# 959AI994/Multi-Gate-VAE

Measured on AMD Instinct MI355X. Metric: circuit-graphs/sec (train step), AIG-64k batch=64 per GPU, higher is better.
Workload: dtype f32 storage; dense products as bf16x3 split-precision MFMA, fp32 accumulate; 1 GPU; cfg2: DG_AE --type aig, 64 x 65536-node synthetic levelised DAGs per GPU (N=4194304, E=6558720, 120 levels), H=64, 4+4 rounds, layernorm, weights [1,4,4], negatives sampled; step includes the 7-scalar metrics copy (pinned, read one step behind); global_batch=64, parallelism=dp1

## Files before the change

### include/mgvae_hip.h

```cpp
#ifndef MGVAE_HIP_H
#define MGVAE_HIP_H
#include <stdint.h>
#ifdef __cplusplus
extern "C" {
#endif

#ifndef MGV_OK
#define MGV_OK 0
#define MGV_EINVAL (-1)
#define MGV_EUNSUPPORTED (-2)
#endif

int mgv_abi_version(void);

int mgv_struct_stage_fwd(int H, int64_t N, const float* h_in, const int32_t* nbr_ptr, const int32_t* nbr_idx,
                         const uint8_t* xcls, const float* xtab, int C, const float* Wc, const float* bc,
                         const float* Whh, const float* bhh, const float* ln_w, const float* ln_b, float ln_eps,
                         float* h_out, void* stream);
int mgv_struct_stage_bwd(int H, int64_t N, const float* h_in, const int32_t* nbr_ptr, const int32_t* nbr_idx,
                         const uint8_t* xcls, const float* xtab, int C, const float* Wc, const float* WcT,
                         const float* bc, const float* Whh, const float* WhhT, const float* bhh,
                         const float* ln_w, const float* ln_b, float ln_eps, const float* gy_direct,
                         const float* gy_agg, float* g_direct_out, float* g_agg_out, float* dWc, float* dbc,
                         float* dWhh, float* dbhh, float* dxtab, float* dln_w, float* dln_b, void* stream);
int mgv_struct_stage_rows_fwd(int H, int64_t N, const float* h_in, const int32_t* nbr_ptr, const int32_t* nbr_idx,
                              const float* xrow, const float* Wc, const float* bc, const float* Whh, const float* bhh,
                              const float* ln_w, const float* ln_b, float ln_eps, float* h_out, void* stream);
int mgv_struct_stage_rows_bwd(int H, int64_t N, const float* h_in, const int32_t* nbr_ptr, const int32_t* nbr_idx,
                              const float* xrow, const float* Wc, const float* WcT, const float* bc, const float* Whh,
                              const float* WhhT, const float* bhh, const float* ln_w, const float* ln_b, float ln_eps,
                              const float* gy_direct, const float* gy_agg, float* g_direct_out, float* g_agg_out,
                              float* dWc, float* dbc, float* dWhh, float* dbhh, float* d_xrow, float* dln_w, float* dln_b,
                              void* stream);

int mgv_struct_stage_fwd_x3(int H, int64_t N, const float* h_in, const int32_t* nbr_ptr, const int32_t* nbr_idx,
                            const uint8_t* xcls, const float* xtab, int C, const void* wpack_bf16, const float* bc,
                            const float* bhh, const float* ln_w, const float* ln_b, float ln_eps, float* h_out,
                            int heavy_n, const int32_t* heavy_nodes, float* heavy_ws, const int32_t* table_own_idx,
                            int nbr_tagged, float* ln_stats_out, void* stream);
int mgv_struct_stage_bwd_x3(int H, int64_t N, const float* h_in, const int32_t* nbr_ptr, const int32_t* nbr_idx,
                            const uint8_t* xcls, const float* xtab, int C, const void* wpack_bf16, const float* bc,
                            const float* bhh, const float* ln_w, const float* ln_b, float ln_eps,
                            const float* gy_direct, const float* gy_agg, float* g_direct_out, float* g_agg_out,
                            float* dWc, float* dbc, float* dWhh, float* dbhh, float* dxtab, float* dln_w,
                            float* dln_b, int heavy_n, const int32_t* heavy_nodes, float* heavy_ws, const int32_t* table_own_idx,
                            int nbr_tagged, void* stream);

int mgv_struct_stage_bwd2_ws_floats(int H, int64_t N);
int mgv_struct_stage_bwd2_x3(int H, int64_t N, const float* h_in, const int32_t* nbr_ptr, const int32_t* nbr_idx,
                             const uint8_t* xcls, const float* xtab, int C, const void* wpack_bf16, const float* bc,
                             const float* bhh, const float* ln_w, const float* ln_b, float ln_eps,
                             const float* gy_direct, const float* gy_agg, float* g_direct_out, float* g_agg_out,
                             float* dWc, float* dbc, float* dWhh, float* dbhh, float* dxtab, float* dln_w,
                             float* dln_b, float* workspace, int64_t workspace_floats, int heavy_n,
                             const int32_t* heavy_nodes, float* heavy_ws, const int32_t* table_own_idx,
                             int nbr_tagged, const float* ln_stats, void* stream);

int mgv_linear_fwd(int64_t N, const float* X1, int K1, int ld1, const float* X2, int K2, int ld2,
                   const float* W, const float* b, int M, float* Y, int ldy, void* stream);
int mgv_linear_wgrad(int64_t N, const float* X1, int K1, int ld1, const float* X2, int K2, int ld2,
                     const float* dY, int lddy, int M, float* dW, float* db, void* stream);
int mgv_linear_x3_supported(int M, int K);
int mgv_wpack_bf16x3(const float* W, int R, int K, int ldw, int transpose, void* hi, void* lo, void* stream);
int mgv_linear_fwd_x3(int64_t N, const float* X1, int K1, int ld1, const float* X2, int K2, int ld2,
                      const void* wpack_bf16, const float* b, int M, float* Y, int ldy, void* stream);
int mgv_grouped_linear_supported(int M, int K);
int mgv_grouped_linear_fwd_x3(int64_t ntiles, const int32_t* tile_list, const int32_t* order, const int32_t* tile_start,
                              const int32_t* tile_count, const int32_t* tile_slot, const float* X, int K, int ldx,
                              const void* wpack_bf16, const float* b, int M, const float* R, int ldr, float* Y, int ldy, void* stream);
int mgv_grouped_linear_wgrad_x3_ws_floats(int M, int K, int64_t ntiles);
int mgv_grouped_linear_wgrad_x3(int64_t ntiles, const int32_t* tile_list, const int32_t* order, const int32_t* tile_start,
                                const int32_t* tile_count, const float* X, int K, int ldx, const float* dY, int lddy, int M,
                                float* dW, float* db, float* workspace, int64_t workspace_floats, void* stream);
int mgv_linear_fwd_x3_res(int64_t N, const float* X1, int K1, int ld1, const float* X2, int K2, int ld2,
                          const void* wpack_bf16, const float* b, int M, const float* R, int ldr, float* Y, int ldy,
                          void* stream);
int mgv_linear_wgrad_x3_ws_floats(int M, int K, int64_t N);
int mgv_linear_wgrad_x3(int64_t N, const float* X1, int K1, int ld1, const float* X2, int K2, int ld2,
                        const float* dY, int lddy, int M, float* dW, float* db, float* workspace, int64_t workspace_floats,
                        void* stream);
int mgv_linear_bwd_x3_supported(int M, int K);
int mgv_linear_bwd_x3(int64_t N, const float* X1, int K1, int ld1, const float* X2, int K2, int ld2, const float* dY, int lddy,
                      int M, const void* wtpack_bf16, float* dW, float* db, float* dX1, int ldx1, float* dX2, int ldx2,
                      const float* R, int ldr, float* workspace, int64_t workspace_floats, void* stream);
int mgv_gather_sum(int H, int64_t N, const float* h, const int32_t* nbr_ptr, const int32_t* nbr_idx,
                   float* agg, float* deg, void* stream);

int mgv_class_expand(int H, int64_t N, const float* table, const int32_t* class_id, float* out, void* stream);
int mgv_seg_sum(int H, int64_t n_seg, const int32_t* seg_ptr, const int32_t* items, const float* direct, const float* agg,
                const int32_t* nbr_ptr, const int32_t* nbr_idx, const int32_t* out_row, float* out, void* stream);
int mgv_seg_sum_entries(int H, int64_t n_seg, const int32_t* seg_ptr, const int32_t* entries, const float* direct, const float* agg,
                        const int32_t* out_row, float* out, void* stream);

int mgv_class_pull_sum_ws_floats(int H, int64_t N, int C);
int mgv_class_pull_sum(int H, int64_t N, const float* gy_direct, const float* gy_agg, const int32_t* nbr_ptr,
                       const int32_t* nbr_idx, const int32_t* class_id, int C, float* out, float* workspace,
                       int64_t workspace_floats, void* stream);

int mgv_func_sweep_fwd(int H, int64_t N, int T, int num_levels, const int32_t* level_tile_ptr_host,
                       const int32_t* order, const int32_t* tile_start, const int32_t* tile_count,
                       const int32_t* tile_slot, const int32_t* in_ptr, const int32_t* in_src, const float* hs,
                       float* hf, const float* attn_u, const float* Wvc, const float* bvc, const float* bih,
                       const float* bhh, const float* gh, const float* h_prev, void* stream);
int mgv_func_sweep_bwd(int H, int64_t N, int T, int num_levels, const int32_t* level_tile_ptr_host,
                       const int32_t* order, const int32_t* tile_start, const int32_t* tile_count,
                       const int32_t* tile_slot, const int32_t* in_ptr, const int32_t* in_src,
                       const int32_t* out_ptr, const int32_t* out_dst, const int32_t* out_slot,
                       const uint8_t* gslot, const float* hs, const float* hf, const float* attn_u,
                       const float* Wvc, const float* WvcT, const float* bvc, const float* bih, const float* bhh,
                       const float* ghf, float* ghs, float* dzb, float* alpha, float* dsc, float* d_attn_u,
                       float* dWvc, float* dbvc, float* dbih, float* dbhh, const float* gh, const float* h_prev,
                       float* d_gh, float* g_hprev, void* stream);

int mgv_sweep_zero_inactive(int H, int64_t N, const uint8_t* gslot, float* hf, void* stream);
int mgv_func_sweep_fwd_x3(int H, int64_t N, int T, int num_levels, const int32_t* level_tile_ptr_host,
                          const int32_t* order, const int32_t* order_span, int order_span_ints, const int32_t* tile_start,
                          const int32_t* tile_count, const int32_t* tile_slot, const int32_t* in_ptr,
                          const int32_t* in_src, const float* hs, float* hf, const float* attn_u,
                          const void* wpack_bf16, const float* bvc, const float* bih, const float* bhh,
                          const float* gh, const float* h_prev, void* stream);
int mgv_func_sweep_bwd_x3(int H, int64_t N, int T, int num_levels, const int32_t* level_tile_ptr_host,
                          const int32_t* order, const int32_t* order_span, int order_span_ints, int64_t n_active,
                          const int32_t* tile_start, const int32_t* tile_count, const int32_t* tile_slot,
                          const int32_t* slot_tiles, const int32_t* slot_tile_ptr_host, const int32_t* in_ptr,
                          const int32_t* in_src, const int32_t* out_ptr, const int32_t* out_dst,
                          const int32_t* out_slot, const uint8_t* gslot, const float* hs, const float* hf,
                          const float* attn_u, const void* wpack_bf16, const float* bvc, const float* bih,
                          const float* bhh, const float* ghf, float* ghs, float* dzb, float* alpha, float* dsc,
                          float* d_attn_u, float* dWvc, float* dbvc, float* dbih, float* dbhh, float* scratch,
                          int64_t scratch_elems,
                          int skip_inactive_longer_than ,
                          int heavy_active_n, const int32_t* heavy_nodes, const int32_t* heavy_node_seg_ptr, const int32_t* heavy_seg_e0,
                          const int32_t* heavy_seg_e1, const int32_t* heavy_lvl_k_ptr_host, const int32_t* heavy_lvl_seg_ptr_host,
                          float* heavy_ws, int skip_active_longer_than,
                          const float* gh, const float* h_prev, float* d_gh, float* g_hprev, void* stream);

int mgv_attn_pool_fwd(int W, int64_t N, const int32_t* in_ptr, const int32_t* in_src, const float* x, const float* u,
                      float* zbar, float* mstat, float* inv, void* stream);
int mgv_attn_pool_bwd(int W, int64_t N, const int32_t* in_ptr, const int32_t* in_src, const float* x, const float* u,
                      const float* zbar, const float* mstat, const float* inv, const float* dzbar, float* dx, float* du,
                      void* stream);

int mgv_sweep_pull_heavy(int H, int K, const int32_t* nodes, const int32_t* node_seg_ptr, int S, const int32_t* seg_e0,
                         const int32_t* seg_e1, const int32_t* out_dst, const int32_t* out_slot, const uint8_t* gslot,
                         const float* alpha, const float* dsc, const float* dzb, const float* attn_u, float* partial_ws,
                         float* ghs, void* stream);

int mgv_edge_dot_fwd(int H, int64_t E, const float* s, const float* t, int ld, const int64_t* src,
                     const int64_t* dst, int sigmoid, float* out, void* stream);
int mgv_edge_dot_bwd(int H, int64_t E, const float* s, const float* t, int ld, const int64_t* src,
                     const int64_t* dst, int sigmoid, const float* gout, float* ds, float* dt, void* stream);
int mgv_pair_scores_fwd(int H, int64_t M, int64_t N, const float* s, int lds, const float* t, int ldt, int sigmoid, float* out,
                        int64_t ldo, void* stream);
int mgv_pair_scores_bwd(int H, int64_t M, int64_t N, const float* s, int lds, const float* t, int ldt, int sigmoid, const float* out,
                        int64_t ldo, const float* gout, int64_t ldg, float* ds, int ldds, float* dt, int lddt, void* stream);
int mgv_pair_scores_at(int H, int64_t E, const float* s, int lds, const float* t, int ldt, const int64_t* src, const int64_t* dst,
                       int sigmoid, float* out, void* stream);
int mgv_pair_topk(int H, int64_t N, const float* s, int lds, const float* t, int ldt, const int32_t* graph_ptr, int G, int k, int sigmoid,
                  float threshold, int skip_self, int32_t* idx, float* score, int32_t* n_above, void* stream);
int mgv_pair_select_count(int H, int64_t N, const float* s, int lds, const float* t, int ldt, const int32_t* graph_ptr, int G, int sigmoid,
                          float threshold, int skip_self, int32_t* n_sel, void* stream);
int mgv_pair_select_fill(int H, int64_t N, const float* s, int lds, const float* t, int ldt, const int32_t* graph_ptr, int G, int sigmoid,
                         float threshold, int skip_self, const int64_t* row_ptr, int64_t cap, int32_t* col, float* score, void* stream);
int mgv_row_unit(int H, int64_t N, const float* x, int ldx, float eps, float* y, int ldy, float* norm, void* stream);
int mgv_sim_select_count(int H, int64_t N, const float* y, int ldy, const int32_t* graph_ptr, int G, float threshold, int32_t* n_sel,
                         void* stream);
int mgv_sim_select_fill(int H, int64_t N, const float* y, int ldy, const int32_t* graph_ptr, int G, float threshold,
                        const int64_t* row_ptr, int64_t cap, int32_t* col, float* score, void* stream);
int mgv_pair_hist(int H, int64_t N, const float* s, int lds, const float* t, int ldt, const int32_t* graph_ptr, int G, int sigmoid,
                  int skip_self, const float* edges, int B, int64_t* hist, void* stream);
int mgv_sim_hist(int H, int64_t N, const float* y, int ldy, const int32_t* graph_ptr, int G, const float* edges, int B, int64_t* hist,
                 void* stream);
int mgv_pair_rank_counts(int H, int64_t N, const float* s, int lds, const float* t, int ldt, const int32_t* graph_ptr, int G, int skip_self,
                         const int32_t* thr_ptr, const float* thr, int32_t* n_gt, int32_t* n_eq, void* stream);
int mgv_cc_init(int64_t N, int32_t* parent, int32_t* status, void* stream);
int mgv_cc_union_pairs(int64_t N, int64_t P, const int64_t* a, const int64_t* b, int32_t* parent, int32_t* status, void* stream);
int mgv_cc_labels(int64_t N, int32_t* parent, int32_t* label, int32_t* size, void* stream);
int mgv_cc_class_ws_ints(int64_t N);
int mgv_cc_class_count(int64_t N, const int32_t* label, int min_size, const int32_t* status, int32_t* ws, int64_t ws_ints, int32_t* counts,
                       void* stream);
int mgv_cc_class_fill(int64_t N, const int32_t* label, int64_t C, int64_t M, int32_t* ws, int64_t ws_ints, void* sort_temp,
                      int64_t sort_temp_ints, int64_t* class_ptr, int32_t* members, void* stream);
int mgv_sim_union(int H, int64_t N, const float* y, int ldy, const int32_t* graph_ptr, int G, float threshold, int32_t* parent,
                  int32_t* status, void* stream);
int mgv_recon_loss_fwd(int H, const float* s, const float* t, int ld, const int64_t* pos_src, const int64_t* pos_dst,
                       int64_t Epos, const int64_t* neg_src, const int64_t* neg_dst, int64_t Eneg,
                       double* sums, uint64_t* counts, int32_t* pred_bin, double* workspace, int64_t workspace_doubles,
                       void* stream);
int mgv_recon_loss_bwd(int H, int64_t N, const float* s, const float* t, int ld, const int64_t* pos_src, const int64_t* pos_dst,
                       int64_t Epos, const int32_t* pos_out_ptr, const int32_t* pos_out_dst, const int32_t* pos_in_ptr,
                       const int32_t* pos_in_src, const int64_t* neg_src, const int64_t* neg_dst, int64_t Eneg,
                       const float* gscale, float* ds, float* dt, void* stream);
int mgv_recon_loss_bwd_csr(int H, int64_t N, const float* s, const float* t, int ld, const int32_t* pos_out_ptr,
                           const int32_t* pos_out_dst, const int32_t* pos_in_ptr, const int32_t* pos_in_src, int64_t Epos,
                           const int32_t* neg_out_ptr, const int32_t* neg_out_dst, const int32_t* neg_in_ptr,
                           const int32_t* neg_in_src, int64_t Eneg, const float* gscale, float* ds, float* dt,
                           int skip_pos_longer_than , void* stream);
int mgv_recon_heavy_lists(int H, const float* s, const float* t, int ld, int64_t Epos, const float* gscale, int K,
                          const int32_t* nodes, const int32_t* node_seg_ptr, int S, const int32_t* seg_node, const int32_t* seg_e0,
                          const int32_t* seg_e1, const int32_t* list, int which, float* partial_ws, float* out, void* stream);
int mgv_recon_step_csr(int H, int64_t N, const float* s, const float* t, int ld, const int32_t* pos_out_ptr,
                       const int32_t* pos_out_dst, const int32_t* pos_in_ptr, const int32_t* pos_in_src, int64_t Epos,
                       const int32_t* neg_out_ptr, const int32_t* neg_out_dst, const int32_t* neg_in_ptr,
                       const int32_t* neg_in_src, int64_t Eneg, float expect_scale, double* sums, uint64_t* counts, float* ds,
                       float* dt, int skip_pos_longer_than, double* workspace, int64_t workspace_doubles, void* stream);
int mgv_recon_step_heavy_lists(int H, const float* s, const float* t, int ld, int64_t Epos, float expect_scale, int K,
                               const int32_t* nodes, const int32_t* node_seg_ptr, int S, const int32_t* seg_node,
                               const int32_t* seg_e0, const int32_t* seg_e1, const int32_t* list, int which, float* partial_ws,
                               float* out, double* sums, uint64_t* counts, double* workspace, int64_t workspace_doubles,
                               void* stream);
int mgv_rows_rescale_unless(int64_t n_floats, float* rows, const float* g_dev, float expect_scale, void* stream);
int mgv_link_keys(int H, const float* s, const float* t, int ld, const int64_t* pos_src, const int64_t* pos_dst, int64_t P,
                  const int64_t* neg_src, const int64_t* neg_dst, int64_t Q, uint32_t* keys, float* scores, int32_t* status,
                  void* stream);
int mgv_link_rank_work_ints(int64_t n);
int mgv_link_rank(int64_t n, int64_t P, const uint32_t* sorted_keys, const int32_t* order, double* out, int32_t* work,
                  int64_t work_ints, void* stream);
int mgv_neg_sample(int64_t N, int64_t E, uint64_t seed, const int32_t* pos_out_ptr, const int32_t* pos_out_dst,
                   int64_t* neg_src, int64_t* neg_dst, int32_t* cnt_out, int32_t* cnt_in, int32_t* rank_out, int32_t* rank_in,
                   void* stream);
int mgv_neg_bucket(int64_t E, const int64_t* neg_src, const int64_t* neg_dst, const int32_t* out_ptr, const int32_t* in_ptr,
                   const int32_t* rank_out, const int32_t* rank_in, int64_t* srt_src, int64_t* srt_dst, int32_t* out_dst, int32_t* in_src,
                   void* stream);

int mgv_func_loss_fwd(int H, int64_t P, const float* hf, const int64_t* pair_a, const int64_t* pair_b,
                      const float* tt, float eps, float* dis, double* ws, double* workspace, int64_t workspace_doubles,
                      void* stream);
int mgv_func_loss_bwd_csr(int H, int64_t N, int64_t P, const float* hf, const int64_t* pair_a, const int64_t* pair_b, const float* tt_sim,
                          const float* dis, float eps, const double* workspace8, const float* grad_loss, const int32_t* a_ptr,
                          const int32_t* a_pair, const int32_t* b_ptr, const int32_t* b_pair, const float* add, float* dhf, void* stream);
int mgv_func_loss_bwd(int H, int64_t P, const float* hf, const int64_t* pair_a, const int64_t* pair_b,
                      const float* tt, const float* dis, float eps, const double* ws, const float* gscale,
                      float* dhf, void* stream);
int mgv_concord_counts(int64_t P, const float* gt, const float* pred, const int32_t* seg_ptr, int G, const float* gaps_host, int B,
                       int64_t* out, void* stream);

int mgv_reparam_fwd(int64_t n, const float* mu, const float* logstd, const float* eps, uint64_t seed,
                    float* eps_out, float* z, double* klsum, void* stream);
int mgv_reparam_bwd(int64_t n, const float* mu, const float* logstd, const float* eps, const float* gz,
                    const float* gkl, float klcoef, float* dmu, float* dlogstd, void* stream);
int mgv_confusion(int64_t n, const int32_t* pred_bin, const int32_t* gt_bin, uint64_t* counts, void* stream);

int mgv_sum_workspace_doubles(void);
int mgv_colstats(int64_t N, int C, const float* Y, int ld, double* sums, double* workspace, int64_t workspace_doubles, void* stream);
int mgv_bn_act_fwd(int64_t N, int C, const float* Y, const float* mean, const float* invstd, const float* gamma,
                   const float* beta, float p_drop, uint64_t seed, float* A, void* stream);
int mgv_bn_act_bwd(int64_t N, int C, const float* Y, const float* mean, const float* invstd, const float* gamma,
                   const float* beta, float p_drop, uint64_t seed, const float* dA, float* dZ, double* sums, double* workspace,
                   int64_t workspace_doubles, void* stream);
int mgv_bn_bwd_apply(int64_t N, int C, const float* Y, const float* mean, const float* invstd, const float* gamma,
                     const float* dZ, const double* sums, int batch_stats, float* dY, void* stream);
int mgv_readout_head_fwd(int64_t N, int C, const float* A, const float* w, const float* b, int clamp01, float* prob, void* stream);
int mgv_readout_head_bwd(int64_t N, int C, const float* A, const float* w, const float* b, int clamp01, const float* dprob,
                         float* dA, float* dw, float* db, double* workspace, int64_t workspace_doubles, void* stream);
int mgv_readout_fused_pack_elems(void);
int mgv_readout_fused_grad_floats(void);
int mgv_readout_fused_ws_doubles(int64_t N);
int mgv_readout_fused_fwd(int64_t N, const float* hf, const void* wpack, const float* b1, const float* g1, const float* be1,
                          float* rm1, float* rv1, const float* b2, const float* g2, const float* be2, float* rm2, float* rv2,
                          const float* w3, const float* b3, float p1, float p2, uint64_t seed1, uint64_t seed2, float momentum,
                          float keep, float eps, int clamp01, float* y1, float* y2, float* stats, double* sums, float* prob,
                          double* workspace, int64_t workspace_doubles, void* stream);
int mgv_readout_fused_bwd(int64_t N, const float* hf, const float* y1, const float* y2, const float* stats, const float* dprob,
                          const void* wpack, const float* g1, const float* be1, const float* g2, const float* be2, const float* w3,
                          const float* b3, float p1, float p2, uint64_t seed1, uint64_t seed2, int clamp01, float* dhf,
                          float* grads, double* sums, double* workspace, int64_t workspace_doubles, void* stream);
int mgv_l1_loss_fwd(int64_t n, const float* x, const float* target, double* sum, double* workspace, int64_t workspace_doubles,
                    void* stream);
int mgv_l1_loss_bwd(int64_t n, const float* x, const float* target, const float* gscale, float* dx, void* stream);

int mgv_adam_step(int64_t n, float* param, const float* grad, float* exp_avg, float* exp_avg_sq, float lr,
                  float beta1, float beta2, float eps, float weight_decay, float grad_scale, int64_t step, void* stream);

int mgv_scan_exclusive_i32(int64_t n, const int32_t* in, int32_t* out, int32_t* scratch, void* stream);
int mgv_plan_csr_scratch_ints(int64_t N, int64_t E);
int mgv_plan_csr(int64_t N, int64_t E, const int64_t* src, const int64_t* dst, int32_t* in_ptr, int32_t* in_src, int32_t* in_dst,
                 int32_t* out_ptr, int32_t* out_dst, int32_t* out_slot, int32_t* in_eid ,
                 int32_t* out_eid , int32_t* scratch, int64_t scratch_ints, int32_t* status, void* stream);
int mgv_sort_lists_i32(int64_t N, int64_t E, const int32_t* ptr, int32_t* vals, int32_t* scratch, int64_t scratch_ints, void* stream);
int mgv_plan_levels(int64_t N, const int32_t* in_ptr, const int32_t* out_ptr, const int32_t* out_dst, int32_t* level, int rounds,
                    int32_t* scratch, int64_t scratch_ints, int32_t* done, void* stream);
int mgv_plan_keys(int64_t N, int T, const float* gate, const int64_t* level64, const uint8_t* slot_of_gate_host256, uint8_t* gslot,
                  int32_t* level32, int32_t* key, int32_t* maxlevel, void* stream);
int mgv_plan_check_levels(int64_t E, const int32_t* in_src, const int32_t* in_dst, const uint8_t* gslot, const int32_t* level, int32_t* err,
                          void* stream);
int mgv_count_sort_scratch_ints(int64_t n, int K);
int mgv_count_sort_i32(int64_t n, const int32_t* key, int K, int32_t* order, int32_t* key_start, int32_t* scratch, int64_t scratch_ints,
                       void* stream);
int mgv_plan_tile_counts(int K, const int32_t* key_start, int32_t* ntile, int32_t* tile_first, int32_t* scan_scratch, void* stream);
int mgv_plan_tiles(int K, int T, int L, int64_t n_active, const int32_t* key_start, const int32_t* tile_first, const int32_t* order,
                   const int32_t* in_ptr, const int32_t* out_ptr, int32_t* tile_start, int32_t* tile_count, int32_t* tile_slot,
                   int32_t* order_span, int32_t* level_tile_ptr, void* stream);
int mgv_plan_order_rows(int64_t n_active, const int32_t* order, const int32_t* in_ptr, const int32_t* in_src, const int32_t* out_ptr,
                        const int32_t* out_dst, const int32_t* out_slot, const uint8_t* gslot, int32_t* rows, void* stream);
int mgv_plan_pairs(int64_t N, const int32_t* in_ptr, const uint8_t* xcls, int32_t* present, int32_t* rank, int32_t* scan_scratch, int32_t* cid,
                   int32_t* cls_deg, uint8_t* cls_x, int32_t* status, void* stream);

int mgv_colour_keys(int64_t N, const int32_t* nbr_ptr, const int32_t* nbr_idx, const int32_t* prev, const int64_t* f, int64_t fstride,
                    const uint8_t* xcls, int key_bits, int64_t* key, void* stream);
int mgv_colour_check(int64_t N, const int32_t* nbr_ptr, const int32_t* nbr_idx, const int32_t* prev, const uint8_t* xcls, const int32_t* cid,
                     const int32_t* rep, int32_t* flags, void* stream);
int mgv_sort_pairs_temp_ints(int key_bytes, int64_t n);
int mgv_sort_pairs(int key_bytes, int64_t n, const void* keys_in, void* keys_out, int32_t* order, int end_bit, void* temp,
                   int64_t temp_ints, void* stream);
int mgv_colour_groups(int64_t N, const int64_t* skey, const int32_t* by_colour, int32_t* cid, int32_t* starts, int32_t* rep, int32_t* n_colours,
                      int32_t* scratch, int64_t scratch_ints, void* stream);
int mgv_colour_rep_rows(int64_t C, const int32_t* rep, const int32_t* nbr_ptr, const int32_t* prev, const uint8_t* xcls, int heavy_row,
                        int32_t* rptr, int32_t* own, uint8_t* xrep, int32_t* n_heavy, int32_t* scratch, int64_t scratch_ints, void* stream);
int mgv_colour_rep_lists(int64_t C, const int32_t* rep, const int32_t* nbr_ptr, const int32_t* nbr_idx, const int32_t* prev, const int32_t* rptr,
                         int32_t* ent, int32_t* row, void* stream);
int mgv_sorted_key_counts(int64_t n, const int32_t* sorted_keys, int64_t K, int32_t* counts, void* stream);
int mgv_seg_level_work_ints(int64_t G);
int mgv_seg_level_scan(int64_t G, const int32_t* counts, int seg, int32_t* work, int64_t work_ints, void* stream);
int mgv_seg_level_fill(int64_t G, int64_t n_seg, const int32_t* gid, int seg, int base, const int32_t* work, int32_t* seg_ptr, int32_t* out_row,
                       int32_t* gid_next, int32_t* counts_next, void* stream);
int mgv_seg_entries_scratch_ints(int64_t n_items);
int mgv_seg_entries(int64_t n_items, const int32_t* items, const int32_t* nbr_ptr, const int32_t* nbr_idx, int64_t n_seg, const int32_t* seg_ptr,
                    int64_t n_entries, int32_t* entries, int32_t* ent_seg_ptr, int32_t* scratch, int64_t scratch_ints, void* stream);

int mgv_digcn_scales(int64_t N, const int32_t* list_ptr, const int32_t* opp_ptr, float alpha, float beta, int self_loops,
                     float* r, float* c, void* stream);
int mgv_digcn_gather(int H, int64_t N, const float* y, const int32_t* nbr_ptr, const int32_t* nbr_idx, const float* outer,
                     const float* inner, const float* mask, int self_loops, int relu, int heavy_n, const int32_t* heavy_nodes,
                     float* out, void* stream);
int mgv_digcn_class_fwd(int H, int64_t N, const uint8_t* xcls, const float* T, int C, const int32_t* nbr_ptr, const int32_t* nbr_idx,
                        const float* outer, const float* inner, int self_loops, int relu, float* out, void* stream);
int mgv_digcn_class_bwd_ws_floats(int H, int64_t N);
int mgv_digcn_class_bwd(int H, int64_t N, const uint8_t* xcls, int C, const int32_t* nbr_ptr, const int32_t* nbr_idx, const float* outer,
                        const float* inner, int self_loops, const float* z, const float* dz, float* dT, float* workspace,
                        int64_t workspace_floats, void* stream);

#ifdef __cplusplus
}
#endif
#endif
```

### multi-gate-vae_amd/csrc/neg_sample.hip

```cpp
#include "mgv_common.h"
#include "../../include/mgvae_hip.h"

namespace mgv {

__device__ __forceinline__ uint64_t splitmix64(uint64_t x) {
    x += 0x9E3779B97F4A7C15ull;
    x = (x ^ (x >> 30)) * 0xBF58476D1CE4E5B9ull;
    x = (x ^ (x >> 27)) * 0x94D049BB133111EBull;
    return x ^ (x >> 31);
}

__global__ __launch_bounds__(kThreads) void k_neg_sample(int64_t N, int64_t E, uint64_t seed, const int32_t* out_ptr, const int32_t* out_dst,
                                                        int64_t* neg_src, int64_t* neg_dst, int32_t* cnt_out, int32_t* cnt_in,
                                                        int32_t* rank_out, int32_t* rank_in) {
    for (int64_t i = (int64_t)blockIdx.x * kThreads + threadIdx.x; i < E; i += (int64_t)gridDim.x * kThreads) {
        uint64_t ctr = seed ^ ((uint64_t)i * 0xD1342543DE82EF95ull);
        int s, d;
        for (int attempt = 0;; ++attempt) {
            const uint64_t r = splitmix64(ctr + attempt);
            s = (int)(((r >> 32) * (uint64_t)N) >> 32);
            d = (int)(((r & 0xFFFFFFFFull) * (uint64_t)N) >> 32);
            bool ok = s != d;
            if (ok)
                for (int e = out_ptr[s]; e < out_ptr[s + 1]; ++e)
                    if (out_dst[e] == d) { ok = false; break; }
            if (ok || attempt >= 64) break;
        }
        neg_src[i] = s; neg_dst[i] = d;
        rank_out[i] = atomicAdd(cnt_out + s, 1);
        rank_in[i] = atomicAdd(cnt_in + d, 1);
    }
}

__global__ __launch_bounds__(kThreads) void k_neg_bucket(int64_t E, const int64_t* neg_src, const int64_t* neg_dst, const int32_t* out_ptr,
                                                        const int32_t* in_ptr, const int32_t* rank_out, const int32_t* rank_in, int64_t* srt_src,
                                                        int64_t* srt_dst, int32_t* out_dst, int32_t* in_src) {
    for (int64_t i = (int64_t)blockIdx.x * kThreads + threadIdx.x; i < E; i += (int64_t)gridDim.x * kThreads) {
        const int s = (int)neg_src[i], d = (int)neg_dst[i];
        const int p = out_ptr[s] + rank_out[i];
        srt_src[p] = s; srt_dst[p] = d; out_dst[p] = d;
        in_src[in_ptr[d] + rank_in[i]] = s;
    }
}

}

extern "C" int mgv_neg_sample(int64_t N, int64_t E, uint64_t seed, const int32_t* pos_out_ptr, const int32_t* pos_out_dst,
                              int64_t* neg_src, int64_t* neg_dst, int32_t* cnt_out, int32_t* cnt_in, int32_t* rank_out, int32_t* rank_in,
                              void* stream) {
    MGV_CHECK_ARG(N >= 2 && N < (1ll << 31) && E >= 0 && pos_out_ptr && cnt_out && cnt_in && rank_out && rank_in);
    if (E == 0) return MGV_OK;
    MGV_CHECK_ARG(neg_src && neg_dst);
    hipLaunchKernelGGL(mgv::k_neg_sample, dim3(mgv::grid_for((E + mgv::kThreads - 1) / mgv::kThreads, 16)), dim3(mgv::kThreads), 0,
                       static_cast<hipStream_t>(stream), N, E, seed, pos_out_ptr, pos_out_dst, neg_src, neg_dst, cnt_out, cnt_in, rank_out, rank_in);
    MGV_LAUNCH_RET();
}

extern "C" int mgv_neg_bucket(int64_t E, const int64_t* neg_src, const int64_t* neg_dst, const int32_t* out_ptr, const int32_t* in_ptr,
                              const int32_t* rank_out, const int32_t* rank_in, int64_t* srt_src, int64_t* srt_dst, int32_t* out_dst, int32_t* in_src,
                              void* stream) {
    MGV_CHECK_ARG(E >= 0 && out_ptr && in_ptr && rank_out && rank_in);
    if (E == 0) return MGV_OK;
    MGV_CHECK_ARG(neg_src && neg_dst && srt_src && srt_dst && out_dst && in_src);
    hipLaunchKernelGGL(mgv::k_neg_bucket, dim3(mgv::grid_for((E + mgv::kThreads - 1) / mgv::kThreads, 16)), dim3(mgv::kThreads), 0,
                       static_cast<hipStream_t>(stream), E, neg_src, neg_dst, out_ptr, in_ptr, rank_out, rank_in, srt_src, srt_dst, out_dst, in_src);
    MGV_LAUNCH_RET();
}
```

### multi-gate-vae_amd/deepgate/sampling.py

```python
import itertools

import torch

from . import _hip
from ._hip import ptr

_CALLS = itertools.count()


class NegativeEdges:

    def __init__(self, edge_index, out_ptr, out_dst, in_ptr, in_src):
        self.edge_index, self.out_ptr, self.out_dst, self.in_ptr, self.in_src = edge_index, out_ptr, out_dst, in_ptr, in_src

    @property
    def csr(self):
        return self.out_ptr, self.out_dst, self.in_ptr, self.in_src


def bucket_negatives(neg, N):
    dev = neg.device
    E = int(neg.shape[1])
    i32 = dict(dtype=torch.int32, device=dev)
    src, dst = neg[0].contiguous(), neg[1].contiguous()
    in_ptr, out_ptr = torch.empty(N + 1, **i32), torch.empty(N + 1, **i32)
    in_src, in_dst, out_dst, out_slot = (torch.empty(max(E, 1), **i32) for _ in range(4))
    n_s = _hip.call_value('mgv_plan_csr_scratch_ints', N, E)
    scratch = torch.empty(n_s, **i32)
    status = torch.empty(2, **i32)
    _hip.call('mgv_plan_csr', N, E, ptr(src), ptr(dst), ptr(in_ptr), ptr(in_src), ptr(in_dst), ptr(out_ptr), ptr(out_dst), ptr(out_slot),
              None, None, ptr(scratch), n_s, ptr(status))
    if int(status[0].item()) != 0:
        raise ValueError('neg_edge_index holds node ids outside [0, num_nodes)')
    counts = (out_ptr[1:] - out_ptr[:-1]).long()
    srt_src = torch.repeat_interleave(torch.arange(N, device=dev), counts, output_size=E)
    srt = torch.stack([srt_src, out_dst[:E].long()])
    return NegativeEdges(srt, out_ptr, out_dst, in_ptr, in_src)


def negative_sampling_device(plan, num_neg_samples=None, generator=None):
    N, dev = plan.N, plan.device
    if getattr(plan, 'num_self_loops', None) is None:
        plan.count_self_loops()
    E = (plan.E - plan.num_self_loops) + N if num_neg_samples is None else int(num_neg_samples)
    base = generator.initial_seed() if generator is not None else torch.initial_seed()
    seed = (base * 0x9E3779B97F4A7C15 + next(_CALLS) * 0xD1B54A32D192ED03 + 0x2545F4914F6CDD1D) & 0xFFFFFFFFFFFFFFFF
    scratch = torch.zeros(2, N, dtype=torch.int32, device=dev)
    neg = torch.empty(2, E, dtype=torch.int64, device=dev)
    rank = torch.empty(2, max(E, 1), dtype=torch.int32, device=dev)
    _hip.call('mgv_neg_sample', N, E, seed, ptr(plan.out_ptr), ptr(plan.out_dst), ptr(neg[0]), ptr(neg[1]), ptr(scratch[0]), ptr(scratch[1]),
              ptr(rank[0]), ptr(rank[1]))
    ptrs = torch.zeros(2, N + 1, dtype=torch.int32, device=dev)
    for k in range(2):
        ptrs[k, 1:] = torch.cumsum(scratch[k], 0, dtype=torch.int32)
    srt = torch.empty(2, E, dtype=torch.int64, device=dev)
    out_dst = torch.empty(max(E, 1), dtype=torch.int32, device=dev)
    in_src = torch.empty(max(E, 1), dtype=torch.int32, device=dev)
    _hip.call('mgv_neg_bucket', E, ptr(neg[0]), ptr(neg[1]), ptr(ptrs[0]), ptr(ptrs[1]), ptr(rank[0]), ptr(rank[1]),
              ptr(srt[0]), ptr(srt[1]), ptr(out_dst), ptr(in_src))
    ss = torch.empty(N + 1 + E, dtype=torch.int32, device=dev)
    _hip.call('mgv_sort_lists_i32', N, E, ptr(ptrs[0]), ptr(out_dst), ptr(ss), ss.numel())
    _hip.call('mgv_sort_lists_i32', N, E, ptr(ptrs[1]), ptr(in_src), ptr(ss), ss.numel())
    srt[1].copy_(out_dst[:E])
    return NegativeEdges(srt, ptrs[0], out_dst, ptrs[1], in_src)


def sorted_edge_keys(pos_edge_index, num_nodes):
    src, dst = pos_edge_index[0].long(), pos_edge_index[1].long()
    keep = src != dst
    return torch.sort(src[keep] * int(num_nodes) + dst[keep]).values


def negative_sampling(pos_edge_index, num_nodes, num_neg_samples=None, generator=None, keys=None):
    dev = pos_edge_index.device
    N = int(num_nodes)
    if keys is None:
        keys = sorted_edge_keys(pos_edge_index, N)
    want = int(keys.numel()) + N if num_neg_samples is None else int(num_neg_samples)
    out = torch.empty((2, 0), dtype=torch.long, device=dev)
    guard = 0
    while out.shape[1] < want:
        m = want - out.shape[1]
        m = m + m // 8 + 16
        s = torch.randint(0, N, (m,), device=dev, generator=generator)
        d = torch.randint(0, N, (m,), device=dev, generator=generator)
        k = s * N + d
        ok = s != d
        if keys.numel() > 0:
            pos = torch.searchsorted(keys, k).clamp_(max=keys.numel() - 1)
            ok &= keys[pos] != k
        out = torch.cat([out, torch.stack([s[ok], d[ok]])], dim=1)
        guard += 1
        if guard > 64:
            raise RuntimeError('negative_sampling: graph too dense to draw %d non-edges' % want)
    return out[:, :want].contiguous()
```

Before: 1047 graphs/s.

## Build negative-edge CSR via chunked radix partition instead of global atomics and sorts

```diff
diff --git a/include/mgvae_hip.h b/include/mgvae_hip.h
--- a/include/mgvae_hip.h
+++ b/include/mgvae_hip.h
@@ -222,6 +222,10 @@
 int mgv_neg_bucket(int64_t E, const int64_t* neg_src, const int64_t* neg_dst, const int32_t* out_ptr, const int32_t* in_ptr,
                    const int32_t* rank_out, const int32_t* rank_in, int64_t* srt_src, int64_t* srt_dst, int32_t* out_dst, int32_t* in_src,
                    void* stream);
+int mgv_neg_partition_ws_ints(int64_t N, int64_t E);
+int mgv_neg_partition(int64_t N, int64_t E, uint64_t seed, int shift, const int32_t* pos_out_ptr, const int32_t* pos_out_dst,
+                      int64_t* edge_index, int32_t* out_ptr, int32_t* out_dst, int32_t* in_ptr, int32_t* in_src, int32_t* ws,
+                      int64_t ws_ints, void* stream);
 
 int mgv_func_loss_fwd(int H, int64_t P, const float* hf, const int64_t* pair_a, const int64_t* pair_b,
                       const float* tt, float eps, float* dis, double* ws, double* workspace, int64_t workspace_doubles,
diff --git a/multi-gate-vae_amd/csrc/mgv_neg_draw.h b/multi-gate-vae_amd/csrc/mgv_neg_draw.h
--- /dev/null
+++ b/multi-gate-vae_amd/csrc/mgv_neg_draw.h
@@ -0,0 +1,27 @@
+#pragma once
+#include "mgv_common.h"
+
+namespace mgv {
+
+__device__ __forceinline__ uint64_t splitmix64(uint64_t x) {
+    x += 0x9E3779B97F4A7C15ull;
+    x = (x ^ (x >> 30)) * 0xBF58476D1CE4E5B9ull;
+    x = (x ^ (x >> 27)) * 0x94D049BB133111EBull;
+    return x ^ (x >> 31);
+}
+
+__device__ __forceinline__ void neg_draw_slot(int64_t N, uint64_t seed, int64_t i, const int32_t* out_ptr, const int32_t* out_dst, int& s, int& d) {
+    uint64_t ctr = seed ^ ((uint64_t)i * 0xD1342543DE82EF95ull);
+    for (int attempt = 0;; ++attempt) {
+        const uint64_t r = splitmix64(ctr + attempt);
+        s = (int)(((r >> 32) * (uint64_t)N) >> 32);
+        d = (int)(((r & 0xFFFFFFFFull) * (uint64_t)N) >> 32);
+        bool ok = s != d;
+        if (ok)
+            for (int e = out_ptr[s]; e < out_ptr[s + 1]; ++e)
+                if (out_dst[e] == d) { ok = false; break; }
+        if (ok || attempt >= 64) break;
+    }
+}
+
+}
diff --git a/multi-gate-vae_amd/csrc/neg_partition.hip b/multi-gate-vae_amd/csrc/neg_partition.hip
--- /dev/null
+++ b/multi-gate-vae_amd/csrc/neg_partition.hip
@@ -0,0 +1,278 @@
+#include "mgv_launch.h"
+#include "mgv_neg_draw.h"
+#include "../../include/mgvae_hip.h"
+
+namespace mgv {
+
+constexpr int kNpChunk = 16384;
+constexpr int kNpDrawThreads = 512;
+constexpr int kNpThreads = 1024;
+constexpr int kNpMaxBlocks = 2048;
+constexpr int kNpMaxShift = 12;
+constexpr int kNpCap = 16384;
+constexpr int kNpShort = 32;
+constexpr int kNpScanInts = 17;
+constexpr int64_t kNpMaxE = 1ll << 28;
+
+__device__ __forceinline__ void np_exscan(int* a, int n, int* s_w) {
+    const int lane = threadIdx.x & 63, w = threadIdx.x >> 6;
+    if (threadIdx.x == 0) s_w[16] = 0;
+    __syncthreads();
+    for (int b0 = 0; b0 < n; b0 += kNpThreads) {
+        const int i = b0 + threadIdx.x;
+        const int t = i < n ? a[i] : 0;
+        int inc = t;
+#pragma unroll
+        for (int d = 1; d < 64; d <<= 1) { const int u = __shfl_up(inc, d, 64); if (lane >= d) inc += u; }
+        if (lane == 63) s_w[w] = inc;
+        __syncthreads();
+        int woff = s_w[16];
+        for (int k = 0; k < w; ++k) woff += s_w[k];
+        if (i < n) a[i] = woff + inc - t;
+        __syncthreads();
+        if (threadIdx.x == kNpThreads - 1) s_w[16] = woff + inc;
+        __syncthreads();
+    }
+    if (threadIdx.x == 0) a[n] = s_w[16];
+    __syncthreads();
+}
+
+__device__ __forceinline__ void np_sort_wide(int32_t* a, int n) {
+    for (unsigned k = 2; (k >> 1) < (unsigned)n; k <<= 1) {
+        for (unsigned i = threadIdx.x; i < (unsigned)n; i += blockDim.x) {
+            const unsigned j = i ^ (k - 1);
+            if (j > i && j < (unsigned)n) { const int x = a[i], y = a[j]; if (y < x) { a[i] = y; a[j] = x; } }
+        }
+        __syncthreads();
+        for (unsigned h = k >> 2; h > 0; h >>= 1) {
+            for (unsigned i = threadIdx.x; i < (unsigned)n; i += blockDim.x) {
+                const unsigned j = i ^ h;
+                if (j > i && j < (unsigned)n) { const int x = a[i], y = a[j]; if (y < x) { a[i] = y; a[j] = x; } }
+            }
+            __syncthreads();
+        }
+    }
+}
+
+__global__ __launch_bounds__(kNpDrawThreads) void k_np_draw(int64_t N, int64_t E, uint64_t seed, const int32_t* pos_ptr, const int32_t* pos_dst,
+                                                            int shift, int nb, int nchunks, int32_t* ps, int32_t* pd, int32_t* hist) {
+    __shared__ int s_h[2 * kNpMaxBlocks];
+    for (int b = threadIdx.x; b < 2 * nb; b += kNpDrawThreads) s_h[b] = 0;
+    __syncthreads();
+    const int64_t c0 = (int64_t)blockIdx.x * kNpChunk;
+    const int64_t c1 = c0 + kNpChunk < E ? c0 + kNpChunk : E;
+    for (int64_t i = c0 + threadIdx.x; i < c1; i += kNpDrawThreads) {
+        int s, d;
+        neg_draw_slot(N, seed, i, pos_ptr, pos_dst, s, d);
+        ps[i] = s; pd[i] = d;
+        atomicAdd(&s_h[s >> shift], 1);
+        atomicAdd(&s_h[nb + (d >> shift)], 1);
+    }
+    __syncthreads();
+    for (int b = threadIdx.x; b < 2 * nb; b += kNpDrawThreads) hist[(int64_t)b * nchunks + blockIdx.x] = s_h[b];
+}
+
+__global__ __launch_bounds__(kNpThreads) void k_np_partition(int64_t E, int shift, int nb, int nchunks, const int32_t* ps, const int32_t* pd,
+                                                             const int32_t* base, int2* part0, int2* part1) {
+    extern __shared__ __attribute__((aligned(16))) int s_dyn[];
+    int2* s_pair = reinterpret_cast<int2*>(s_dyn);
+    int* s_cur = s_dyn + 2 * kNpChunk;
+    int* s_delta = s_cur + nb + 1;
+    int* s_w = s_delta + nb;
+    constexpr int PT = kNpChunk / kNpThreads;
+    const int64_t c0 = (int64_t)blockIdx.x * kNpChunk;
+    const int m = (int)((c0 + kNpChunk < E ? c0 + kNpChunk : E) - c0);
+    int rs[PT], rd[PT];
+#pragma unroll
+    for (int j = 0; j < PT; ++j) {
+        const int i = j * kNpThreads + threadIdx.x;
+        rs[j] = i < m ? ps[c0 + i] : 0;
+        rd[j] = i < m ? pd[c0 + i] : 0;
+    }
+    for (int side = 0; side < 2; ++side) {
+        for (int b = threadIdx.x; b < nb; b += kNpThreads) s_cur[b] = 0;
+        __syncthreads();
+#pragma unroll
+        for (int j = 0; j < PT; ++j)
+            if (j * kNpThreads + (int)threadIdx.x < m) atomicAdd(&s_cur[(side ? rd[j] : rs[j]) >> shift], 1);
+        __syncthreads();
+        np_exscan(s_cur, nb, s_w);
+        for (int b = threadIdx.x; b < nb; b += kNpThreads)
+            s_delta[b] = base[((int64_t)side * nb + b) * nchunks + blockIdx.x] - (side ? (int)E : 0) - s_cur[b];
+        __syncthreads();
+#pragma unroll
+        for (int j = 0; j < PT; ++j)
+            if (j * kNpThreads + (int)threadIdx.x < m) {
+                const int k = side ? rd[j] : rs[j], o = side ? rs[j] : rd[j];
+                s_pair[atomicAdd(&s_cur[k >> shift], 1)] = make_int2(k, o);
+            }
+        __syncthreads();
+        int2* part = side ? part1 : part0;
+        for (int p = threadIdx.x; p < m; p += kNpThreads) {
+            const int2 pr = s_pair[p];
+            part[s_delta[pr.x >> shift] + p] = pr;
+        }
+        __syncthreads();
+    }
+}
+
+__global__ __launch_bounds__(kNpThreads) void k_np_finish(int64_t N, int64_t E, int shift, int nb, int nchunks, const int32_t* base,
+                                                          const int2* part0, const int2* part1, int32_t* out_ptr, int32_t* out_dst,
+                                                          int32_t* in_ptr, int32_t* in_src, int64_t* ei0, int64_t* ei1, int32_t* status) {
+    extern __shared__ __attribute__((aligned(16))) int s_dyn[];
+    const int L = 1 << shift;
+    int* s_val = s_dyn;
+    int* s_ptr = s_dyn + kNpCap;
+    int* s_cur = s_ptr + L + 1;
+    int* s_w = s_cur + L + 1;
+    int& s_n = s_w[kNpScanInts];
+    const int b = blockIdx.x, side = blockIdx.y, tid = threadIdx.x;
+    const int2* part = side ? part1 : part0;
+    int32_t* gptr = side ? in_ptr : out_ptr;
+    int32_t* list = side ? in_src : out_dst;
+    const int64_t hb = ((int64_t)side * nb + b) * nchunks;
+    const int off = side ? (int)E : 0;
+    const int start = base[hb] - off, n = base[hb + nchunks] - off - start;
+    const int64_t node0 = (int64_t)b << shift;
+    const int nodes = (int)(N - node0 < L ? N - node0 : L);
+    part += start;
+
+    for (int i = tid; i < nodes; i += kNpThreads) s_ptr[i] = 0;
+    __syncthreads();
+    for (int i = tid; i < n; i += kNpThreads) atomicAdd(&s_ptr[part[i].x - (int)node0], 1);
+    __syncthreads();
+    np_exscan(s_ptr, nodes, s_w);
+    for (int i = tid; i < nodes; i += kNpThreads) gptr[node0 + i] = start + s_ptr[i];
+    if (b == nb - 1 && tid == 0) gptr[N] = start + n;
+
+    int trips = 0, wide = 0;
+    for (int lo = 0; lo < nodes; ++trips) {
+        const int p0 = s_ptr[lo];
+        int hi = lo + 1;
+        if (s_ptr[hi] - p0 > kNpCap) {
+            const int len = s_ptr[hi] - p0;
+            int32_t* row = list + start + p0;
+            if (tid == 0) s_n = 0;
+            __syncthreads();
+            for (int i = tid; i < n; i += kNpThreads) {
+                const int2 pr = part[i];
+                if (pr.x - (int)node0 == lo) row[atomicAdd(&s_n, 1)] = pr.y;
+            }
+            __syncthreads();
+            np_sort_wide(row, len);
+            if (!side)
+                for (int p = tid; p < len; p += kNpThreads) { ei0[start + p0 + p] = node0 + lo; ei1[start + p0 + p] = row[p]; }
+            __syncthreads();
+            ++wide;
+        } else {
+            int z = nodes;
+            while (hi < z) { const int mid = (hi + z + 1) >> 1; if (s_ptr[mid] - p0 <= kNpCap) hi = mid; else z = mid - 1; }
+            const int m = s_ptr[hi] - p0;
+            for (int i = lo + tid; i < hi; i += kNpThreads) s_cur[i] = s_ptr[i] - p0;
+            if (tid == 0) s_n = 0;
+            __syncthreads();
+            for (int i = tid; i < n; i += kNpThreads) {
+                const int2 pr = part[i];
+                const int k = pr.x - (int)node0;
+                if (k >= lo && k < hi) s_val[atomicAdd(&s_cur[k], 1)] = pr.y;
+            }
+            __syncthreads();
+            for (int i = lo + tid; i < hi; i += kNpThreads) {
+                int* v = s_val + (s_ptr[i] - p0);
+                const int len = s_ptr[i + 1] - s_ptr[i];
+                if (len > kNpShort) { s_cur[atomicAdd(&s_n, 1)] = i; continue; }
+                for (int a = 1; a < len; ++a) {
+                    const int x = v[a];
+                    int c = a;
+                    for (; c > 0 && v[c - 1] > x; --c) v[c] = v[c - 1];
+                    v[c] = x;
+                }
+            }
+            __syncthreads();
+            const int nlong = s_n;
+            for (int q = 0; q < nlong; ++q) {
+                const int i = s_cur[q];
+                np_sort_wide(s_val + (s_ptr[i] - p0), s_ptr[i + 1] - s_ptr[i]);
+            }
+            for (int p = tid; p < m; p += kNpThreads) {
+                const int v = s_val[p];
+                const int64_t g = (int64_t)start + p0 + p;
+                list[g] = v;
+                if (!side) {
+                    int a = lo, c = hi - 1;
+                    while (a < c) { const int mid = (a + c + 1) >> 1; if (s_ptr[mid] <= p0 + p) a = mid; else c = mid - 1; }
+                    ei0[g] = node0 + a;
+                    ei1[g] = v;
+                }
+            }
+            __syncthreads();
+        }
+        lo = hi;
+    }
+    if (tid == 0) {
+        if (b == 0 && side == 0) status[0] = nb;
+        atomicMax(status + 1, n);
+        atomicAdd(status + 2, trips);
+        atomicAdd(status + 3, wide);
+    }
+}
+
+struct NpLayout { int64_t status, hist, scan, scratch, part0, part1, total; };
+
+static NpLayout np_layout(int64_t E, int64_t nb) {
+    const int64_t nchunks = (E + kNpChunk - 1) / kNpChunk, nh = 2 * nb * nchunks;
+    NpLayout w;
+    w.status = 0;
+    w.hist = 8;
+    w.scan = w.hist + nh;
+    w.scratch = w.scan + nh + 2;
+    w.part0 = (w.scratch + nh / 2048 + 4 + 1) & ~1ll;
+    w.part1 = w.part0 + 2 * E;
+    w.total = w.part1 + 2 * E;
+    return w;
+}
+
+}
+
+using namespace mgv;
+
+extern "C" int mgv_neg_partition_ws_ints(int64_t N, int64_t E) {
+    if (N < 2 || N >= (1ll << 31) || E < 0 || E >= kNpMaxE) return -1;
+    return (int)np_layout(E, kNpMaxBlocks).total;
+}
+
+extern "C" int mgv_neg_partition(int64_t N, int64_t E, uint64_t seed, int shift, const int32_t* pos_out_ptr, const int32_t* pos_out_dst,
+                                 int64_t* edge_index, int32_t* out_ptr, int32_t* out_dst, int32_t* in_ptr, int32_t* in_src, int32_t* ws,
+                                 int64_t ws_ints, void* stream) {
+    MGV_CHECK_ARG(N >= 2 && N < (1ll << 31) && E >= 0 && E < kNpMaxE && pos_out_ptr && out_ptr && in_ptr && ws);
+    MGV_CHECK_ARG((reinterpret_cast<uintptr_t>(ws) & 7) == 0 && ws_ints >= mgv_neg_partition_ws_ints(N, E));
+    MGV_CHECK_ARG(E == 0 || (edge_index && out_dst && in_src));
+    if (shift < 0 || shift > kNpMaxShift) return MGV_EUNSUPPORTED;
+    const int64_t L = 1ll << shift, nb64 = (N + L - 1) / L;
+    if (nb64 > kNpMaxBlocks) return MGV_EUNSUPPORTED;
+    hipStream_t st = static_cast<hipStream_t>(stream);
+    hipMemsetAsync(ws, 0, 8 * sizeof(int32_t), st);
+    if (E == 0) {
+        hipMemsetAsync(out_ptr, 0, (N + 1) * sizeof(int32_t), st);
+        hipMemsetAsync(in_ptr, 0, (N + 1) * sizeof(int32_t), st);
+        MGV_LAUNCH_RET();
+    }
+    const int nb = (int)nb64, nchunks = (int)((E + kNpChunk - 1) / kNpChunk);
+    const NpLayout w = np_layout(E, nb);
+    int32_t* ps = reinterpret_cast<int32_t*>(edge_index);
+    int32_t* pd = ps + E;
+    int2* part0 = reinterpret_cast<int2*>(ws + w.part0);
+    int2* part1 = reinterpret_cast<int2*>(ws + w.part1);
+    hipLaunchKernelGGL(k_np_draw, dim3(nchunks), dim3(kNpDrawThreads), 0, st, N, E, seed, pos_out_ptr, pos_out_dst, shift, nb, nchunks, ps, pd,
+                       ws + w.hist);
+    const int rc = mgv_scan_exclusive_i32(2ll * nb * nchunks, ws + w.hist, ws + w.scan, ws + w.scratch, stream);
+    if (rc != MGV_OK) return rc;
+    const size_t lds_b = (size_t)(2 * kNpChunk + 2 * nb + 1 + kNpScanInts) * sizeof(int);
+    allow_lds<k_np_partition>();
+    hipLaunchKernelGGL(k_np_partition, dim3(nchunks), dim3(kNpThreads), lds_b, st, E, shift, nb, nchunks, ps, pd, ws + w.scan, part0, part1);
+    const size_t lds_c = (size_t)(kNpCap + 2 * ((int)L + 1) + kNpScanInts + 1) * sizeof(int);
+    allow_lds<k_np_finish>();
+    hipLaunchKernelGGL(k_np_finish, dim3(nb, 2), dim3(kNpThreads), lds_c, st, N, E, shift, nb, nchunks, ws + w.scan, part0, part1, out_ptr, out_dst,
+                       in_ptr, in_src, edge_index, edge_index + E, ws + w.status);
+    MGV_LAUNCH_RET();
+}
diff --git a/multi-gate-vae_amd/csrc/neg_sample.hip b/multi-gate-vae_amd/csrc/neg_sample.hip
--- a/multi-gate-vae_amd/csrc/neg_sample.hip
+++ b/multi-gate-vae_amd/csrc/neg_sample.hip
@@ -1,31 +1,15 @@
 #include "mgv_common.h"
+#include "mgv_neg_draw.h"
 #include "../../include/mgvae_hip.h"
 
 namespace mgv {
-
-__device__ __forceinline__ uint64_t splitmix64(uint64_t x) {
-    x += 0x9E3779B97F4A7C15ull;
-    x = (x ^ (x >> 30)) * 0xBF58476D1CE4E5B9ull;
-    x = (x ^ (x >> 27)) * 0x94D049BB133111EBull;
-    return x ^ (x >> 31);
-}
 
 __global__ __launch_bounds__(kThreads) void k_neg_sample(int64_t N, int64_t E, uint64_t seed, const int32_t* out_ptr, const int32_t* out_dst,
                                                         int64_t* neg_src, int64_t* neg_dst, int32_t* cnt_out, int32_t* cnt_in,
                                                         int32_t* rank_out, int32_t* rank_in) {
     for (int64_t i = (int64_t)blockIdx.x * kThreads + threadIdx.x; i < E; i += (int64_t)gridDim.x * kThreads) {
-        uint64_t ctr = seed ^ ((uint64_t)i * 0xD1342543DE82EF95ull);
         int s, d;
-        for (int attempt = 0;; ++attempt) {
-            const uint64_t r = splitmix64(ctr + attempt);
-            s = (int)(((r >> 32) * (uint64_t)N) >> 32);
-            d = (int)(((r & 0xFFFFFFFFull) * (uint64_t)N) >> 32);
-            bool ok = s != d;
-            if (ok)
-                for (int e = out_ptr[s]; e < out_ptr[s + 1]; ++e)
-                    if (out_dst[e] == d) { ok = false; break; }
-            if (ok || attempt >= 64) break;
-        }
+        neg_draw_slot(N, seed, i, out_ptr, out_dst, s, d);
         neg_src[i] = s; neg_dst[i] = d;
         rank_out[i] = atomicAdd(cnt_out + s, 1);
         rank_in[i] = atomicAdd(cnt_in + d, 1);
diff --git a/multi-gate-vae_amd/deepgate/sampling.py b/multi-gate-vae_amd/deepgate/sampling.py
--- a/multi-gate-vae_amd/deepgate/sampling.py
+++ b/multi-gate-vae_amd/deepgate/sampling.py
@@ -1,4 +1,5 @@
 import itertools
+import os
 
 import torch
 
@@ -6,6 +7,26 @@
 from ._hip import ptr
 
 _CALLS = itertools.count()
+
+PARTITION = os.environ.get('MGV_NEG_PARTITION', '1') != '0'
+PART_MAX_SHIFT = 12
+PART_MAX_BLOCKS = 2048
+PART_TARGET = 12288
+PART_MAX_E = 1 << 28
+
+
+def partition_shift(N, E):
+    N, E = int(N), int(E)
+    if N < 2 or N >= 1 << 31 or E < 1 or E >= PART_MAX_E:
+        return None
+    s = 0
+    while s < PART_MAX_SHIFT and (N + (1 << s) - 1) >> s > PART_MAX_BLOCKS:
+        s += 1
+    if (N + (1 << s) - 1) >> s > PART_MAX_BLOCKS:
+        return None
+    while s < PART_MAX_SHIFT and E << (s + 1) <= PART_TARGET * N:
+        s += 1
+    return s
 
 
 class NegativeEdges:
@@ -45,6 +66,15 @@
     E = (plan.E - plan.num_self_loops) + N if num_neg_samples is None else int(num_neg_samples)
     base = generator.initial_seed() if generator is not None else torch.initial_seed()
     seed = (base * 0x9E3779B97F4A7C15 + next(_CALLS) * 0xD1B54A32D192ED03 + 0x2545F4914F6CDD1D) & 0xFFFFFFFFFFFFFFFF
+    shift = partition_shift(N, E) if PARTITION else None
+    if shift is not None:
+        i32 = dict(dtype=torch.int32, device=dev)
+        srt = torch.empty(2, E, dtype=torch.int64, device=dev)
+        ptrs, out_dst, in_src = torch.empty(2, N + 1, **i32), torch.empty(E, **i32), torch.empty(E, **i32)
+        ws = torch.empty(_hip.call_value('mgv_neg_partition_ws_ints', N, E), **i32)
+        _hip.call('mgv_neg_partition', N, E, seed, shift, ptr(plan.out_ptr), ptr(plan.out_dst), ptr(srt), ptr(ptrs[0]), ptr(out_dst),
+                  ptr(ptrs[1]), ptr(in_src), ptr(ws), ws.numel())
+        return NegativeEdges(srt, ptrs[0], out_dst, ptrs[1], in_src)
     scratch = torch.zeros(2, N, dtype=torch.int32, device=dev)
     neg = torch.empty(2, E, dtype=torch.int64, device=dev)
     rank = torch.empty(2, max(E, 1), dtype=torch.int32, device=dev)
```

After: 1071 graphs/s, median of 6. 2.3% higher.
